# GewelsJI/MVLT

Measured on AMD Instinct MI355X. Metric: image-text pairs/sec/node, PVT-tiny MVLT pre-train step, higher is better.
Workload: dtype bf16

## Files before the change

mvlt_amd/_lib.py:

```python
import ctypes as C
import os

import torch

_HERE = os.path.dirname(os.path.abspath(__file__))
LIB_PATH = os.environ.get("MVLT_HIP_LIB") or os.path.join(_HERE, "libmvlt_hip.so")


class MVLTError(RuntimeError):
    pass


if not os.path.exists(LIB_PATH):
    raise ImportError(f"{LIB_PATH} is missing: build it with `python -m mvlt_amd.build` (hipcc, gfx950). "
                      "mvlt_amd has no CPU or eager fallback.")
lib = C.CDLL(LIB_PATH)

c_int, c_float, c_void_p, c_long = C.c_int, C.c_float, C.c_void_p, C.c_long


class RowMap(C.Structure):
    _fields_ = [(n, c_int) for n in ("mode", "rows_per_batch", "batch_stride", "offset",
                                     "r", "w_in", "tokens_in", "hw_out", "w_out", "c_seg", "h_in")]

# ... 165 lines not shown
        raise ImportError(f"{LIB_PATH} does not export {_name} (include/mvlt_hip_ext.h): stale build? run python -m mvlt_amd.build")
    _fn = getattr(lib, _name)
    _fn.restype, _fn.argtypes = _res, _args

EXT_VERSION = 1
if lib.mvlt_ext_version() != EXT_VERSION:
    raise ImportError(f"extension mismatch: {LIB_PATH} is version {lib.mvlt_ext_version()}, the binding is version {EXT_VERSION} (stale build? run python -m mvlt_amd.build)")

EMA_PROTOTYPES = {
    "mvlt_ema_version": (_i, []),
    "mvlt_ema_update": (_i, [_vp, _vp, _vp, _l, _f, _f, _vp, _vp]),
    "mvlt_ema_update_buffers": (_i, [_vp, _i, _f, _f, _vp]),
}
for _name, (_res, _args) in EMA_PROTOTYPES.items():
    if not hasattr(lib, _name):
        raise ImportError(f"{LIB_PATH} does not export {_name} (include/mvlt_hip_ema.h): stale build? run python -m mvlt_amd.build")
    _fn = getattr(lib, _name)
    _fn.restype, _fn.argtypes = _res, _args

EMA_VERSION = 1
if lib.mvlt_ema_version() != EMA_VERSION:
    raise ImportError(f"EMA entry points mismatch: {LIB_PATH} is version {lib.mvlt_ema_version()}, the binding is version {EMA_VERSION} (stale build? run python -m mvlt_amd.build)")

DT = {torch.bfloat16: 0, torch.float32: 1}


def last_kernel():
    s = lib.mvlt_last_kernel().decode()
    s = s.replace("(anonymous namespace)::", "")
    if s.startswith("void "):
        s = s[5:]
    depth = 0
    for i, ch in enumerate(s):
        depth += ch == "<"
        depth -= ch == ">"
        if ch == "(" and depth == 0:
            return s[:i]
    return s


def check(rc, what):
    if rc != 0:
        raise MVLTError(f"{what} failed ({rc}): {lib.mvlt_last_error().decode()}")


_raw_stream, _cur_device = torch._C._cuda_getCurrentRawStream, torch._C._cuda_getDevice
# ... 25 lines not shown
```

mvlt_amd/build.py:

```python
import concurrent.futures
import os
import subprocess
import sys

HERE = os.path.dirname(os.path.abspath(__file__))
CSRC = os.path.join(HERE, "csrc")
OBJ = os.path.join(HERE, "csrc", "_obj")
LIB = os.path.join(HERE, "libmvlt_hip.so")
ARCH = "gfx950"
FLAGS = ["--offload-arch=" + ARCH, "-O3", "-std=c++17", "-fPIC", "-ffp-contract=fast", "-Wno-unused-result"]
EXTRA = {"mlp.hip": ["-fno-slp-vectorize"]}


def _sources():
    return sorted(f for f in os.listdir(CSRC) if f.endswith(".hip"))


def source_hash():
    import hashlib
    h = hashlib.sha256()
    files = sorted(os.path.join(CSRC, f) for f in os.listdir(CSRC) if f.endswith((".hip", ".h", ".inc")))
    files += [os.path.join(HERE, "..", "include", h) for h in ("mvlt_hip.h", "mvlt_hip_ext.h", "mvlt_hip_ema.h")]
    for f in files:
        h.update(os.path.basename(f).encode())
        h.update(open(f, "rb").read())
    return h.hexdigest()[:16]


def _deps_mtime():
    hdrs = [os.path.join(CSRC, f) for f in os.listdir(CSRC) if f.endswith((".h", ".inc"))]
    hdrs += [os.path.join(HERE, "..", "include", h) for h in ("mvlt_hip.h", "mvlt_hip_ext.h", "mvlt_hip_ema.h")]
    return max(os.path.getmtime(h) for h in hdrs)


def _compile(src, force, verbose):
    s = os.path.join(CSRC, src)
    o = os.path.join(OBJ, src[:-4] + ".o")
    if not force and os.path.exists(o) and os.path.getmtime(o) >= max(os.path.getmtime(s), _deps_mtime()):
        return o
    cmd = ["hipcc", *FLAGS, *EXTRA.get(src, []), "-c", s, "-o", o]
    if verbose:
        print(" ".join(cmd), flush=True)
    r = subprocess.run(cmd, capture_output=True, text=True)
    if r.returncode != 0:
        raise RuntimeError(f"hipcc failed for {src}:\n{r.stdout}\n{r.stderr}")
    return o


def build(force=False, verbose=False):
    os.makedirs(OBJ, exist_ok=True)
    srcs = _sources()
    with concurrent.futures.ThreadPoolExecutor(max_workers=min(6, len(srcs))) as ex:
        objs = list(ex.map(lambda s: _compile(s, force, verbose), srcs))
    if force or not os.path.exists(LIB) or any(os.path.getmtime(o) > os.path.getmtime(LIB) for o in objs):
# ... 12 lines not shown
```

mvlt_amd/csrc/mim.hip:

```cpp
#include "common.h"
#include "../../include/mvlt_hip.h"

namespace {

constexpr int NT = 256;

template <typename TO> __device__ __forceinline__ void store4(TO* p, const f32x4& v);
template <> __device__ __forceinline__ void store4<bf16>(bf16* p, const f32x4& v) {
  st_g<MVLT_NT_MIM>((bf16x4*)p, bf16x4{(bf16)v[0], (bf16)v[1], (bf16)v[2], (bf16)v[3]});
}
template <> __device__ __forceinline__ void store4<float>(float* p, const f32x4& v) { st_g<MVLT_NT_MIM>((f32x4*)p, v); }
template <typename T> __device__ __forceinline__ f32x4 load4(const T* p);
template <> __device__ __forceinline__ f32x4 load4<float>(const float* p) { return *(const f32x4*)p; }
typedef _Float16 f16x4 __attribute__((ext_vector_type(4)));
template <> __device__ __forceinline__ f32x4 load4<_Float16>(const _Float16* p) {
  const f16x4 v = *(const f16x4*)p;
  return f32x4{(float)v[0], (float)v[1], (float)v[2], (float)v[3]};
}
template <> __device__ __forceinline__ f32x4 load4<bf16>(const bf16* p) {
  const bf16x4 v = *(const bf16x4*)p;
  return f32x4{(float)v[0], (float)v[1], (float)v[2], (float)v[3]};
}

typedef _Float16 f16x8 __attribute__((ext_vector_type(8)));
template <typename T> __device__ __forceinline__ void load8(const T* p, float (&v)[8]);
template <> __device__ __forceinline__ void load8<float>(const float* p, float (&v)[8]) {
  const f32x4 a = *(const f32x4*)p, b = *(const f32x4*)(p + 4);
#pragma unroll
  for (int e = 0; e < 4; ++e) { v[e] = a[e]; v[4 + e] = b[e]; }
}
template <> __device__ __forceinline__ void load8<bf16>(const bf16* p, float (&v)[8]) {
  const bf16x8 a = *(const bf16x8*)p;
#pragma unroll
  for (int e = 0; e < 8; ++e) v[e] = (float)a[e];
}
template <> __device__ __forceinline__ void load8<_Float16>(const _Float16* p, float (&v)[8]) {
  const f16x8 a = *(const f16x8*)p;
#pragma unroll
  for (int e = 0; e < 8; ++e) v[e] = (float)a[e];
}
template <typename TO> __device__ __forceinline__ void store8(TO* p, const float (&v)[8]);
template <> __device__ __forceinline__ void store8<float>(float* p, const float (&v)[8]) {
  st_g<MVLT_NT_MIM>((f32x4*)p, f32x4{v[0], v[1], v[2], v[3]});
  st_g<MVLT_NT_MIM>((f32x4*)(p + 4), f32x4{v[4], v[5], v[6], v[7]});
}
template <> __device__ __forceinline__ void store8<_Float16>(_Float16* p, const float (&v)[8]) {
  f16x8 o;
#pragma unroll
  for (int e = 0; e < 8; ++e) o[e] = (_Float16)v[e];
  st_g<MVLT_NT_MIM>((f16x8*)p, o);
}
template <> __device__ __forceinline__ void store8<bf16>(bf16* p, const float (&v)[8]) {
  bf16x8 o;
#pragma unroll
  for (int e = 0; e < 8; ++e) o[e] = (bf16)v[e];
  st_g<MVLT_NT_MIM>((bf16x8*)p, o);
}

template <int MODE>
__global__ __launch_bounds__(NT) void col_reduce_kernel(const float* z, int ldz, const float* dy, int lddy, const float* mean, const float* rstd,
                                                        int M, int C, float* s1, float* s2) {
  extern __shared__ float sm[];
  for (int i = threadIdx.x; i < 2 * C; i += NT) sm[i] = 0.f;
  __syncthreads();
  const int lane = threadIdx.x & 63, wave = threadIdx.x >> 6;
  constexpr int MAXC = 4;
  float a1[MAXC], a2[MAXC], mu[MAXC], rs[MAXC];
#pragma unroll
  for (int k = 0; k < MAXC; ++k) {
    a1[k] = 0.f; a2[k] = 0.f;
    int c = lane + 64 * k;
    mu[k] = (MODE == 1 && c < C) ? mean[c] : 0.f;
    rs[k] = (MODE == 1 && c < C) ? rstd[c] : 0.f;
  }
  for (long row = (long)blockIdx.x * 4 + wave; row < M; row += (long)gridDim.x * 4) {
#pragma unroll
    for (int k = 0; k < MAXC; ++k) {
      int c = lane + 64 * k;
      if (c < C) {
        float zv = z[row * ldz + c];
// ... 954 lines not shown
```

mvlt_amd/mim.py:

```python
import torch

from . import ops
from .params import pool_zeros
from ._lib import conv3map, rowmap

BN_EPS, BN_MOM = 1e-5, 0.1
STAT_COPIES = 16
CONVS = ("reduction1", "reduction2", "reduction3", "conv_upsample1", "conv_upsample2", "conv_upsample3", "conv_upsample4",
         "conv_upsample5", "conv_concat2", "conv_concat3", "conv4")
_NO_BN_FOLD = False


def _z(shape, dev, dtype=torch.float32):
    return pool_zeros(shape, dtype, dev)


def _e(shape, dev, dtype=torch.float32):
    return torch.empty(shape, device=dev, dtype=dtype)


class MimStep:
    def __init__(self, model, x2, x3, x4, sides, training, need_grad):
        self.m, self.S = model, model.store
        self.dt = model.compute_dtype
        self.dev = x2.device
        self.x = (x2, x3, x4)
        self.B = x2.shape[0]
        self.s1, self.s2, self.s3 = sides
        self.M1, self.M2, self.M3 = (self.B * h * w for h, w in sides)
        self.training = training
        self.need_grad = need_grad
        self.rec = {}
        self.nbt = []
# ... 73 lines not shown
        f = self.rec
        f16 = torch.float16 if (self.training and dt == torch.bfloat16) else torch.float32
        r = self.conv_bn("reduction1", x2, C2, x2.shape[1], s1, C2, ch, M1); low = _e((M1, ch), dev, f16); self.norm(r, low, ch)
        r = self.conv_bn("reduction2", x3, C3, x3.shape[1], s2, C3, ch, M2); mid = _e((M2, ch), dev); self.norm(r, mid, ch)
        r = self.conv_bn("reduction3", x4, C4, x4.shape[1], s3, C4, ch, M3); high = _e((M3, ch), dev); self.norm(r, high, ch)
        uph = self.up2(high, ch, s3, ch)
        HW1, HW2 = s1[0] * s1[1], s2[0] * s2[1]
        cat2 = _e((M2, 2 * ch), dev, dt)
        r = self.conv_bn("conv_upsample1", uph, ch, HW2, s2, ch, ch, M2); cu1o = _e((M2, ch), dev); self.norm(r, cu1o, ch)
        a = _e((M2, ch), dev)
        ops.ew_mul(a, ch, cu1o, ch, mid, ch, M=M2, Cdim=ch, out16=cat2, ld16=2 * ch)
        r = self.conv_bn("conv_upsample4", uph, ch, HW2, s2, ch, ch, M2); self.norm(r, y16=cat2[:, ch:], ld16=2 * ch)
        r = self.conv_bn("conv_concat2", cat2, 2 * ch, HW2, s2, 2 * ch, 2 * ch, M2); c = _e((M2, 2 * ch), dev); self.norm(r, c, 2 * ch)
        cat3 = _e((M1, 3 * ch), dev, dt)
        upm = self.up2(mid, ch, s2, ch)
        r = self.conv_bn("conv_upsample2", upm, ch, HW1, s1, ch, ch, M1); cu2o = _e((M1, ch), dev, f16); self.norm(r, cu2o, ch)
        upa = self.up2(a, ch, s2, ch)
        r = self.conv_bn("conv_upsample3", upa, ch, HW1, s1, ch, ch, M1); cu3o = _e((M1, ch), dev, f16); self.norm(r, cu3o, ch)
        ops.ew_mul(None, 0, cu2o, ch, cu3o, ch, low, ch, M=M1, Cdim=ch, out16=cat3, ld16=3 * ch)
        upc = self.up2(c, 2 * ch, s2, 2 * ch)
        r = self.conv_bn("conv_upsample5", upc, 2 * ch, HW1, s1, 2 * ch, 2 * ch, M1); self.norm(r, y16=cat3[:, ch:], ld16=3 * ch)
        d16 = _e((M1, 3 * ch), dev, dt)
        r = self.conv_bn("conv_concat3", cat3, 3 * ch, HW1, s1, 3 * ch, 3 * ch, M1); self.norm(r, y16=d16, ld16=3 * ch)
        e16 = _e((M1, 3 * ch), dev, dt)
        r = self.conv_bn("conv4", d16, 3 * ch, HW1, s1, 3 * ch, 3 * ch, M1); self.norm(r, y16=e16, ld16=3 * ch)
        sc = _e((M1, 3), dev)
        ops.gemm_nt(e16, S.extra["t2i_head.score.0.weight::W"], sc, M1, 3, 3 * ch, 3 * ch, 3 * ch, 3, bias=S.master("t2i_head.score.0.bias"))
        if target is not None:
            acc = pool_zeros((1,), torch.float32, dev)
            ops.upsample_l1_fwd(sc, 3, B, s1[0], s1[1], 3, 8, target, acc)
            out = (acc / target.numel()).reshape(())
            self.sc, self.target = sc, target
        else:
            out = _e((B, 3, 8 * s1[0], 8 * s1[1]), dev)
            ops.upsample_fwd(sc, 3, B, s1[0], s1[1], 3, 8, out, 0, nchw=True)
        if self.nbt:
            torch._foreach_add_(self.nbt, 1)
            self.nbt = []
        if self.need_grad:
            self.keep = dict(low=low, mid=mid, cu1o=cu1o, cu2o=cu2o, cu3o=cu3o, e16=e16)
        else:
            self.rec = {}
        return out

    def bn_conv_bwd(self, name, dy, lddy, dx=None, lddx=0, accumulate=False, dx_map=None, dx_dtype=torch.float32, need_dx=True):
        S, dev, dt = self.S, self.dev, self.dt
        r = self.rec[name]
        p, M, cin, cout = r["p"], r["M"], r["cin"], r["cout"]
        red = _z((2, cout), dev)
        ops.bn_bwd_reduce(dy, lddy, r["z"], cout, r["mean"], r["rstd"], M, cout, red[0], red[1])
        dz = _e((M, cout), dev, dt)
        ops.bn_bwd_apply(dy, lddy, r["z"], cout, r["mean"], r["rstd"], S.master(p + ".1.weight"), red[0], red[1], M, cout, dz, cout,
                         g_beta=S.grad(p + ".1.bias"), g_gamma=S.grad(p + ".1.weight"))
        from .schedule import conv_wgrad
        conv_wgrad(S, p + ".0.weight", dz, r["xin"], M, cout, 9 * cin, cout, r["ld_in"], r["amap"], 9, cin)
        if not need_dx:
            return None
        gmap = conv3map(r["side"][0], r["side"][1], r["side"][0] * r["side"][1], cout)
        if dx is None:
            dx, lddx = _e((M, cin), dev, dx_dtype), cin
        ops.gemm_nt(dz, S.extra[p + ".0.weight::F"], dx, M, cin, 9 * cout, cout, 9 * cout, lddx, a_map=gmap, c_map=dx_map,
                    R=dx if accumulate else None)
        return dx

    def backward(self, dout, sink=None, dgrad=True):
        S, dev, dt, B = self.S, self.dev, self.dt, self.B
        s1, s2, s3, M1, M2, M3 = self.s1, self.s2, self.s3, self.M1, self.M2, self.M3
        ch = 64
        k = self.keep
        dsc_p = _z((M1, 8), dev, dt)
        if getattr(self, "target", None) is not None:
            ops.upsample_l1_bwd(self.sc, 3, B, s1[0], s1[1], 3, 8, self.target, dout.reshape(1).float().contiguous(), dsc_p, 8)
            self.sc = self.target = None
        else:
            dout = dout.contiguous().float()
            ops.upsample_bwd(dout, 0, True, B, s1[0], s1[1], 3, 8, dsc_p, 8)
        ops.gemm_tn(dsc_p, k["e16"], S.grad("t2i_head.score.0.weight").view(3, 3 * ch), M1, 3, 3 * ch, 8, 3 * ch, 3 * ch,
                    colsum=S.grad("t2i_head.score.0.bias"))
        gd = dt if dt == torch.bfloat16 else torch.float32
        de = _e((M1, 3 * ch), dev, gd)
        ops.gemm_nt(dsc_p, S.extra["t2i_head.score.0.weight::T"], de, M1, 3 * ch, 8, 8, 8, 3 * ch)
        dd = self.bn_conv_bwd("conv4", de, 3 * ch, dx_dtype=gd)
        dcat3 = self.bn_conv_bwd("conv_concat3", dd, 3 * ch, dx_dtype=gd)
        dupc = self.bn_conv_bwd("conv_upsample5", dcat3[:, ch:], 3 * ch, dx_dtype=gd)
        dc = _e((M2, 2 * ch), dev)
        ops.upsample_bwd(dupc, 2 * ch, False, B, s2[0], s2[1], 2 * ch, 2, dc, 2 * ch)
        db = dcat3
        dcu2o, dcu3o, dlow = _e((M1, ch), dev, gd), _e((M1, ch), dev, gd), _e((M1, ch), dev, gd)
        ops.ew_mul3_bwd(db, 3 * ch, k["cu2o"], k["cu3o"], k["low"], ch, dcu2o, dcu3o, dlow, M1, ch)
        dcat2 = _z((M2, 2 * ch), dev)
        dupa = self.bn_conv_bwd("conv_upsample3", dcu3o, ch, dx_dtype=gd)
        ops.upsample_bwd(dupa, ch, False, B, s2[0], s2[1], ch, 2, dcat2, 2 * ch, accumulate=True)
        dupm = self.bn_conv_bwd("conv_upsample2", dcu2o, ch, dx_dtype=gd)
        dmid = _e((M2, ch), dev)
        ops.upsample_bwd(dupm, ch, False, B, s2[0], s2[1], ch, 2, dmid, ch)
        self.bn_conv_bwd("conv_concat2", dc, 2 * ch, dx=dcat2, lddx=2 * ch, accumulate=True)
        duph = self.bn_conv_bwd("conv_upsample4", dcat2[:, ch:], 2 * ch)
        dcu1o = _e((M2, ch), dev)
        ops.ew_mul(dcu1o, ch, dcat2, 2 * ch, k["mid"], ch, M=M2, Cdim=ch)
        ops.ew_mul(dmid, ch, dcat2, 2 * ch, k["cu1o"], ch, M=M2, Cdim=ch, accumulate=True)
        self.bn_conv_bwd("conv_upsample1", dcu1o, ch, dx=duph, lddx=ch, accumulate=True)
        dhigh = _e((M3, ch), dev)
        ops.upsample_bwd(duph, ch, False, B, s3[0], s3[1], ch, 2, dhigh, ch)
        grads = []
        for name, dy, x, side in (("reduction1", dlow, self.x[0], s1), ("reduction2", dmid, self.x[1], s2), ("reduction3", dhigh, self.x[2], s3)):
# ... 39 lines not shown
```

mvlt_amd/ops.py:

```python
import ctypes as C

import torch

from . import _lib as L
from ._lib import DT, check, patchmap, ptr, rowmap, stream_ptr

_ID = rowmap()


def gemm_nt(A, B, C_out, M, N, K, lda, ldb, ldc, *, a_map=None, c_map=None, bias=None, act=0, H=None,
            row_scale=None, rows_per_scale=0, R=None, col_sum=None, col_sumsq=None, col_copies=0, split_k=0, post_ln=None):
    assert A.dtype == B.dtype and A.dtype in DT and (C_out.dtype in DT or (C_out.dtype == torch.float16 and col_sum is not None))
    if bias is not None:
        assert bias.dtype == torch.float32
    if row_scale is not None:
        assert row_scale.dtype == torch.float32
    if R is not None:
        assert R.dtype == C_out.dtype or (R.dtype == torch.float32 and C_out.dtype == torch.bfloat16)
    if H is not None:
        assert H.dtype == C_out.dtype
    if col_sum is not None:
        assert col_sum.dtype == torch.float32 and col_sumsq is not None and col_sumsq.dtype == torch.float32
    a = L.GemmNTArgs(A=ptr(A), B=ptr(B), C=ptr(C_out), M=M, N=N, K=K, lda=lda, ldb=ldb, ldc=ldc,
                     dtype=DT[A.dtype], out_dtype=2 if C_out.dtype == torch.float16 else DT[C_out.dtype], a_map=a_map or _ID, c_map=c_map or _ID,
# ... 272 lines not shown

def bn_norm(z, ldz, mean, rstd, gamma, beta, M, Cdim, y32=None, ld32=0, y16=None, ld16=0):
    check(L.lib.mvlt_bn_norm(ptr(z), ldz, ZDT[z.dtype], ptr(mean), ptr(rstd), ptr(gamma), ptr(beta), M, Cdim, ptr(y32), ld32, ZDT[y32.dtype] if y32 is not None else 1, ptr(y16), ld16,
                             DT[y16.dtype] if y16 is not None else 0, stream_ptr()), "mvlt_bn_norm")


def bn_finalize_norm(z, ldz, s, ss, copies, eps, momentum, mean, rstd, running_mean, running_var, gamma, beta, M, Cdim, y32=None, ld32=0, y16=None, ld16=0):
    assert z.dtype == torch.float16 and (y16 is None or y16.dtype == torch.bfloat16)
    check(L.lib.mvlt_bn_finalize_norm(ptr(z), ldz, ptr(s), ptr(ss), copies, eps, momentum, ptr(mean), ptr(rstd), ptr(running_mean), ptr(running_var), ptr(gamma), ptr(beta), M, Cdim,
                                      ptr(y32), ld32, ZDT[y32.dtype] if y32 is not None else 1, ptr(y16), ld16, stream_ptr()), "mvlt_bn_finalize_norm")


def bn_bwd_reduce(dy, lddy, z, ldz, mean, rstd, M, Cdim, s1, s2):
    assert dy.dtype in DT and z.dtype in ZDT
    check(L.lib.mvlt_bn_bwd_reduce(ptr(dy), lddy, ptr(z), ldz, ZDT[z.dtype], ptr(mean), ptr(rstd), M, Cdim, ptr(s1), ptr(s2), DT[dy.dtype], stream_ptr()), "mvlt_bn_bwd_reduce")


def bn_bwd_apply(dy, lddy, z, ldz, mean, rstd, gamma, s1, s2, M, Cdim, dz16, lddz, g_beta=None, g_gamma=None):
    assert dy.dtype in DT and z.dtype in ZDT
    check(L.lib.mvlt_bn_bwd_apply(ptr(dy), lddy, ptr(z), ldz, ZDT[z.dtype], ptr(mean), ptr(rstd), ptr(gamma), ptr(s1), ptr(s2), M, Cdim, ptr(dz16), lddz,
                                  ptr(g_beta), ptr(g_gamma), DT[dz16.dtype], DT[dy.dtype], stream_ptr()), "mvlt_bn_bwd_apply")


def ew_mul3_bwd(dy, lddy, a, b, c, ld, da, db, dc, M, Cdim):
    assert dy.dtype in DT and da.dtype == db.dtype == dc.dtype == dy.dtype and a.dtype == b.dtype == c.dtype and a.dtype in ZDT
    check(L.lib.mvlt_ew_mul3_bwd(ptr(dy), lddy, ptr(a), ptr(b), ptr(c), ld, ZDT[a.dtype], ptr(da), ptr(db), ptr(dc), M, Cdim, DT[dy.dtype], stream_ptr()), "mvlt_ew_mul3_bwd")


def ew_mul(out, ldo, a, lda, b, ldb, c=None, ldc=0, *, M, Cdim, accumulate=False, out16=None, ld16=0):
    assert a.dtype == b.dtype and (c is None or c.dtype == a.dtype) and a.dtype in ZDT
    check(L.lib.mvlt_ew_mul(ptr(out), ldo, ptr(a), lda, ptr(b), ldb, ptr(c), ldc, ZDT[a.dtype], M, Cdim, 1 if accumulate else 0, ptr(out16), ld16,
                            DT[out16.dtype] if out16 is not None else 0, stream_ptr()), "mvlt_ew_mul")


def upsample_fwd(x, ldx, B, H, W, Cdim, scale, out, ldo, nchw=False):
    check(L.lib.mvlt_upsample_fwd(ptr(x), ldx, B, H, W, Cdim, scale, ptr(out), ldo, DT[out.dtype], 1 if nchw else 0, stream_ptr()), "mvlt_upsample_fwd")


def upsample_bwd(dy, lddy, nchw, B, H, W, Cdim, scale, dx, lddx, accumulate=False):
    assert dy.dtype in DT and dx.dtype in DT
    check(L.lib.mvlt_upsample_bwd(ptr(dy), lddy, 1 if nchw else 0, B, H, W, Cdim, scale, ptr(dx), lddx, 1 if accumulate else 0, DT[dx.dtype],
                                  DT[dy.dtype], stream_ptr()), "mvlt_upsample_bwd")


def upsample_l1_ok(W, scale):
    return W <= 64 and (W * scale) % 4 == 0 and W * scale <= 256
# ... 136 lines not shown
```

Before: 13370.

## Fuse conv4 BatchNorm with the 3-channel score projection in forward and backward

Adds kernels that apply the conv4 BatchNorm and project straight to the 3-channel score map, so the bf16 normalized activation (M x 3ch) is never written and no separate GEMM is launched. In backward, the score-weight gradient, the de = dsc*W^T product and the BN reduce/apply are computed together from z and the 3-wide score gradient. This removes materialising and rereading the wide de and e16 tensors. In exchange the normalize and de terms are recomputed inside the reduce and apply kernels, and the path is limited to bf16 training with C <= 256.

```diff
diff --git a/include/mvlt_hip_mim.h b/include/mvlt_hip_mim.h
--- /dev/null
+++ b/include/mvlt_hip_mim.h
@@ -0,0 +1,25 @@
+#ifndef MVLT_HIP_MIM_H
+#define MVLT_HIP_MIM_H
+#include <stdint.h>
+#ifdef __cplusplus
+extern "C" {
+#endif
+
+#define MVLT_MIM_VERSION 1
+int mvlt_mim_version(void);
+
+int mvlt_bn_finalize_norm_score(const void* z, int ldz, const float* sum, const float* sumsq, int copies, float eps, float momentum, float* mean, float* rstd,
+                                float* running_mean, float* running_var, const float* gamma, const float* beta, const void* w, const float* bias,
+                                long M, int C, float* sc, int ldsc, void* stream);
+
+int mvlt_bn_bwd_reduce_score_scratch(long M, int C);
+int mvlt_bn_bwd_reduce_score(const void* z, int ldz, const void* dsc, int lddsc, const void* wt, const float* mean, const float* rstd, const float* gamma,
+                             const float* beta, long M, int C, float* s1, float* s2, float* g_w, float* g_b, float* scratch, long scratch_floats, void* stream);
+
+int mvlt_bn_bwd_apply_score(const void* dsc, int lddsc, const void* wt, const void* z, int ldz, const float* mean, const float* rstd, const float* gamma,
+                            const float* s1, const float* s2, long M, int C, void* dz, int lddz, float* g_beta, float* g_gamma, void* stream);
+
+#ifdef __cplusplus
+}
+#endif
+#endif
diff --git a/mvlt_amd/_lib.py b/mvlt_amd/_lib.py
--- a/mvlt_amd/_lib.py
+++ b/mvlt_amd/_lib.py
@@ -211,6 +211,23 @@
 if lib.mvlt_ema_version() != EMA_VERSION:
     raise ImportError(f"EMA entry points mismatch: {LIB_PATH} is version {lib.mvlt_ema_version()}, the binding is version {EMA_VERSION} (stale build? run python -m mvlt_amd.build)")
 
+MIM_PROTOTYPES = {
+    "mvlt_mim_version": (_i, []),
+    "mvlt_bn_finalize_norm_score": (_i, [_vp, _i, _vp, _vp, _i, _f, _f, _vp, _vp, _vp, _vp, _vp, _vp, _vp, _vp, _l, _i, _vp, _i, _vp]),
+    "mvlt_bn_bwd_reduce_score_scratch": (_i, [_l, _i]),
+    "mvlt_bn_bwd_reduce_score": (_i, [_vp, _i, _vp, _i, _vp, _vp, _vp, _vp, _vp, _l, _i, _vp, _vp, _vp, _vp, _vp, _l, _vp]),
+    "mvlt_bn_bwd_apply_score": (_i, [_vp, _i, _vp, _vp, _i, _vp, _vp, _vp, _vp, _vp, _l, _i, _vp, _i, _vp, _vp, _vp]),
+}
+for _name, (_res, _args) in MIM_PROTOTYPES.items():
+    if not hasattr(lib, _name):
+        raise ImportError(f"{LIB_PATH} does not export {_name} (include/mvlt_hip_mim.h): stale build? run python -m mvlt_amd.build")
+    _fn = getattr(lib, _name)
+    _fn.restype, _fn.argtypes = _res, _args
+
+MIM_VERSION = 1
+if lib.mvlt_mim_version() != MIM_VERSION:
+    raise ImportError(f"MIM score entry points mismatch: {LIB_PATH} is version {lib.mvlt_mim_version()}, the binding is version {MIM_VERSION} (stale build? run python -m mvlt_amd.build)")
+
 DT = {torch.bfloat16: 0, torch.float32: 1}
 
 
diff --git a/mvlt_amd/build.py b/mvlt_amd/build.py
--- a/mvlt_amd/build.py
+++ b/mvlt_amd/build.py
@@ -20,7 +20,7 @@
     import hashlib
     h = hashlib.sha256()
     files = sorted(os.path.join(CSRC, f) for f in os.listdir(CSRC) if f.endswith((".hip", ".h", ".inc")))
-    files += [os.path.join(HERE, "..", "include", h) for h in ("mvlt_hip.h", "mvlt_hip_ext.h", "mvlt_hip_ema.h")]
+    files += [os.path.join(HERE, "..", "include", h) for h in ("mvlt_hip.h", "mvlt_hip_ext.h", "mvlt_hip_ema.h", "mvlt_hip_mim.h")]
     for f in files:
         h.update(os.path.basename(f).encode())
         h.update(open(f, "rb").read())
@@ -29,7 +29,7 @@
 
 def _deps_mtime():
     hdrs = [os.path.join(CSRC, f) for f in os.listdir(CSRC) if f.endswith((".h", ".inc"))]
-    hdrs += [os.path.join(HERE, "..", "include", h) for h in ("mvlt_hip.h", "mvlt_hip_ext.h", "mvlt_hip_ema.h")]
+    hdrs += [os.path.join(HERE, "..", "include", h) for h in ("mvlt_hip.h", "mvlt_hip_ext.h", "mvlt_hip_ema.h", "mvlt_hip_mim.h")]
     return max(os.path.getmtime(h) for h in hdrs)
 
 
diff --git a/mvlt_amd/csrc/mim.hip b/mvlt_amd/csrc/mim.hip
--- a/mvlt_amd/csrc/mim.hip
+++ b/mvlt_amd/csrc/mim.hip
@@ -1,61 +1,10 @@
 #include "common.h"
+#include "mim_vec.h"
 #include "../../include/mvlt_hip.h"
 
 namespace {
 
 constexpr int NT = 256;
-
-template <typename TO> __device__ __forceinline__ void store4(TO* p, const f32x4& v);
-template <> __device__ __forceinline__ void store4<bf16>(bf16* p, const f32x4& v) {
-  st_g<MVLT_NT_MIM>((bf16x4*)p, bf16x4{(bf16)v[0], (bf16)v[1], (bf16)v[2], (bf16)v[3]});
-}
-template <> __device__ __forceinline__ void store4<float>(float* p, const f32x4& v) { st_g<MVLT_NT_MIM>((f32x4*)p, v); }
-template <typename T> __device__ __forceinline__ f32x4 load4(const T* p);
-template <> __device__ __forceinline__ f32x4 load4<float>(const float* p) { return *(const f32x4*)p; }
-typedef _Float16 f16x4 __attribute__((ext_vector_type(4)));
-template <> __device__ __forceinline__ f32x4 load4<_Float16>(const _Float16* p) {
-  const f16x4 v = *(const f16x4*)p;
-  return f32x4{(float)v[0], (float)v[1], (float)v[2], (float)v[3]};
-}
-template <> __device__ __forceinline__ f32x4 load4<bf16>(const bf16* p) {
-  const bf16x4 v = *(const bf16x4*)p;
-  return f32x4{(float)v[0], (float)v[1], (float)v[2], (float)v[3]};
-}
-
-typedef _Float16 f16x8 __attribute__((ext_vector_type(8)));
-template <typename T> __device__ __forceinline__ void load8(const T* p, float (&v)[8]);
-template <> __device__ __forceinline__ void load8<float>(const float* p, float (&v)[8]) {
-  const f32x4 a = *(const f32x4*)p, b = *(const f32x4*)(p + 4);
-#pragma unroll
-  for (int e = 0; e < 4; ++e) { v[e] = a[e]; v[4 + e] = b[e]; }
-}
-template <> __device__ __forceinline__ void load8<bf16>(const bf16* p, float (&v)[8]) {
-  const bf16x8 a = *(const bf16x8*)p;
-#pragma unroll
-  for (int e = 0; e < 8; ++e) v[e] = (float)a[e];
-}
-template <> __device__ __forceinline__ void load8<_Float16>(const _Float16* p, float (&v)[8]) {
-  const f16x8 a = *(const f16x8*)p;
-#pragma unroll
-  for (int e = 0; e < 8; ++e) v[e] = (float)a[e];
-}
-template <typename TO> __device__ __forceinline__ void store8(TO* p, const float (&v)[8]);
-template <> __device__ __forceinline__ void store8<float>(float* p, const float (&v)[8]) {
-  st_g<MVLT_NT_MIM>((f32x4*)p, f32x4{v[0], v[1], v[2], v[3]});
-  st_g<MVLT_NT_MIM>((f32x4*)(p + 4), f32x4{v[4], v[5], v[6], v[7]});
-}
-template <> __device__ __forceinline__ void store8<_Float16>(_Float16* p, const float (&v)[8]) {
-  f16x8 o;
-#pragma unroll
-  for (int e = 0; e < 8; ++e) o[e] = (_Float16)v[e];
-  st_g<MVLT_NT_MIM>((f16x8*)p, o);
-}
-template <> __device__ __forceinline__ void store8<bf16>(bf16* p, const float (&v)[8]) {
-  bf16x8 o;
-#pragma unroll
-  for (int e = 0; e < 8; ++e) o[e] = (bf16)v[e];
-  st_g<MVLT_NT_MIM>((bf16x8*)p, o);
-}
 
 template <int MODE>
 __global__ __launch_bounds__(NT) void col_reduce_kernel(const float* z, int ldz, const float* dy, int lddy, const float* mean, const float* rstd,
diff --git a/mvlt_amd/csrc/mim_score.hip b/mvlt_amd/csrc/mim_score.hip
--- /dev/null
+++ b/mvlt_amd/csrc/mim_score.hip
@@ -0,0 +1,324 @@
+#include "common.h"
+#include "mim_vec.h"
+#include "../../include/mvlt_hip.h"
+#include "../../include/mvlt_hip_mim.h"
+
+namespace {
+
+constexpr int NT = 256;
+constexpr int RWGS = 256;
+
+__device__ __forceinline__ float bf16_round(float x) { return (float)(bf16)x; }
+__device__ __forceinline__ float de_of(float d0, float d1, float d2, float w0, float w1, float w2) { return bf16_round(d0 * w0 + d1 * w1 + d2 * w2); }
+
+template <int KC>
+__global__ __launch_bounds__(NT) void bn_fin_norm_score_kernel(const _Float16* z, int ldz, const float* sum, const float* sumsq, int copies, long Mstat, float eps, float momentum,
+                                                               float* mean, float* rstd, float* running_mean, float* running_var, const float* gamma, const float* beta,
+                                                               const bf16* w, const float* bias, long M, int C, float* sc, int ldsc) {
+  __shared__ __attribute__((aligned(16))) float s_mu[256], s_rs[256];
+  for (int c = threadIdx.x; c < C; c += NT) {
+    float s1 = 0.f, s2 = 0.f;
+    for (int k = 0; k < copies; ++k) { s1 += sum[(long)k * C + c]; s2 += sumsq[(long)k * C + c]; }
+    const float m = s1 / (int)Mstat;
+    const float var = fmaxf(s2 / (int)Mstat - m * m, 0.f);
+    const float r = rsqrtf(var + eps);
+    s_mu[c] = m; s_rs[c] = r;
+    if (blockIdx.x == 0) {
+      mean[c] = m; rstd[c] = r;
+      if (running_mean) {
+        running_mean[c] = (1.f - momentum) * running_mean[c] + momentum * m;
+        const float unb = Mstat > 1 ? var * ((float)(int)Mstat / (float)((int)Mstat - 1)) : var;
+        running_var[c] = (1.f - momentum) * running_var[c] + momentum * unb;
+      }
+    }
+  }
+  __syncthreads();
+  const int lane = threadIdx.x & 63, wave = threadIdx.x >> 6, sub = lane & 7;
+  float mu[KC][8], rs[KC][8], ga[KC][8], be[KC][8], w0[KC][8], w1[KC][8], w2[KC][8];
+  bool on[KC];
+#pragma unroll
+  for (int k = 0; k < KC; ++k) {
+    const int c = (sub + 8 * k) * 8;
+    on[k] = c < C;
+    if (on[k]) {
+      load8<float>(s_mu + c, mu[k]); load8<float>(s_rs + c, rs[k]); load8<float>(gamma + c, ga[k]); load8<float>(beta + c, be[k]);
+      load8<bf16>(w + c, w0[k]); load8<bf16>(w + C + c, w1[k]); load8<bf16>(w + 2 * (long)C + c, w2[k]);
+    } else {
+#pragma unroll
+      for (int e = 0; e < 8; ++e) { mu[k][e] = rs[k][e] = ga[k][e] = be[k][e] = w0[k][e] = w1[k][e] = w2[k][e] = 0.f; }
+    }
+  }
+  const float bj = sub < 3 ? bias[sub] : 0.f;
+  constexpr int RPW = NT / 64 * 8;
+  const long stride = (long)gridDim.x * RPW;
+  for (long rb = (long)blockIdx.x * RPW + wave * 8; rb < M; rb += 2 * stride) {
+    float v[2][KC][8];
+#pragma unroll
+    for (int u = 0; u < 2; ++u) {
+      const long r = rb + u * stride + (lane >> 3);
+#pragma unroll
+      for (int k = 0; k < KC; ++k) {
+        if (on[k] && r < M) load8<_Float16>(z + r * ldz + (sub + 8 * k) * 8, v[u][k]);
+        else {
+#pragma unroll
+          for (int e = 0; e < 8; ++e) v[u][k][e] = 0.f;
+        }
+      }
+    }
+#pragma unroll
+    for (int u = 0; u < 2; ++u) {
+      float a0 = 0.f, a1 = 0.f, a2 = 0.f;
+#pragma unroll
+      for (int k = 0; k < KC; ++k)
+#pragma unroll
+        for (int e = 0; e < 8; ++e) {
+          const float o = bf16_round((v[u][k][e] - mu[k][e]) * rs[k][e] * ga[k][e] + be[k][e]);
+          a0 += o * w0[k][e]; a1 += o * w1[k][e]; a2 += o * w2[k][e];
+        }
+#pragma unroll
+      for (int o = 1; o < 8; o <<= 1) { a0 += __shfl_xor(a0, o); a1 += __shfl_xor(a1, o); a2 += __shfl_xor(a2, o); }
+      const long r = rb + u * stride + (lane >> 3);
+      if (sub < 3 && r < M) sc[r * ldsc + sub] = (sub == 0 ? a0 : sub == 1 ? a1 : a2) + bj;
+    }
+  }
+}
+
+template <int NT>
+__global__ __launch_bounds__(NT) void bn_bwd_reduce_score_kernel(const _Float16* z, int ldz, const bf16* dsc, int lddsc, const bf16* wt, const float* mean, const float* rstd,
+                                                                 long M, int C, float* part, int rows_per_wg) {
+  extern __shared__ float sm[];
+  const int lane = threadIdx.x & 63, wave = threadIdx.x >> 6;
+  const int G = (C + 63) >> 6, g = wave % G, wr = wave / G, R = NT / 64 / G, Cp = G * 64;
+  const int rpp = R * 8;
+  const int tc = g * 64 + (lane & 7) * 8, tr = wr * 8 + (lane >> 3);
+  const bool on = tc < C;
+  float a1[8], a2[8], t0[8], t1[8], t2[8], sd[3] = {0.f, 0.f, 0.f};
+  float mu[8], rs[8], w0[8], w1[8], w2[8];
+#pragma unroll
+  for (int e = 0; e < 8; ++e) { a1[e] = a2[e] = t0[e] = t1[e] = t2[e] = 0.f; mu[e] = rs[e] = w0[e] = w1[e] = w2[e] = 0.f; }
+  if (on) {
+    load8<float>(mean + tc, mu);
+    load8<float>(rstd + tc, rs);
+#pragma unroll
+    for (int e = 0; e < 8; ++e) {
+      const bf16x4 q = *(const bf16x4*)(wt + (long)(tc + e) * 8);
+      w0[e] = (float)q[0]; w1[e] = (float)q[1]; w2[e] = (float)q[2];
+    }
+    const long r0 = (long)blockIdx.x * rows_per_wg;
+    const long r1 = (r0 + rows_per_wg < M) ? r0 + rows_per_wg : M;
+    long r = r0 + tr;
+    constexpr int U = 3;
+    for (; r + (long)(U - 1) * rpp < r1; r += (long)U * rpp) {
+      float zv[U][8];
+      bf16x4 dv[U];
+#pragma unroll
+      for (int u = 0; u < U; ++u) {
+        load8<_Float16>(z + (r + (long)u * rpp) * ldz + tc, zv[u]);
+        dv[u] = *(const bf16x4*)(dsc + (r + (long)u * rpp) * lddsc);
+      }
+#pragma unroll
+      for (int u = 0; u < U; ++u) {
+        const float d0 = (float)dv[u][0], d1 = (float)dv[u][1], d2 = (float)dv[u][2];
+        sd[0] += d0; sd[1] += d1; sd[2] += d2;
+#pragma unroll
+        for (int e = 0; e < 8; ++e) {
+          const float xh = (zv[u][e] - mu[e]) * rs[e], de = de_of(d0, d1, d2, w0[e], w1[e], w2[e]);
+          a1[e] += de; a2[e] += de * xh; t0[e] += d0 * xh; t1[e] += d1 * xh; t2[e] += d2 * xh;
+        }
+      }
+    }
+    for (; r < r1; r += rpp) {
+      float zv[8];
+      load8<_Float16>(z + r * ldz + tc, zv);
+      const bf16x4 dv = *(const bf16x4*)(dsc + r * lddsc);
+      const float d0 = (float)dv[0], d1 = (float)dv[1], d2 = (float)dv[2];
+      sd[0] += d0; sd[1] += d1; sd[2] += d2;
+#pragma unroll
+      for (int e = 0; e < 8; ++e) {
+        const float xh = (zv[e] - mu[e]) * rs[e], de = de_of(d0, d1, d2, w0[e], w1[e], w2[e]);
+        a1[e] += de; a2[e] += de * xh; t0[e] += d0 * xh; t1[e] += d1 * xh; t2[e] += d2 * xh;
+      }
+    }
+  }
+#pragma unroll
+  for (int o = 8; o < 64; o <<= 1) {
+#pragma unroll
+    for (int e = 0; e < 8; ++e) {
+      a1[e] += __shfl_xor(a1[e], o); a2[e] += __shfl_xor(a2[e], o);
+      t0[e] += __shfl_xor(t0[e], o); t1[e] += __shfl_xor(t1[e], o); t2[e] += __shfl_xor(t2[e], o);
+    }
+#pragma unroll
+    for (int j = 0; j < 3; ++j) sd[j] += __shfl_xor(sd[j], o);
+  }
+  float* ss = sm + R * 5 * Cp;
+  if (lane < 8) {
+    float* row = sm + (long)wr * 5 * Cp + tc;
+#pragma unroll
+    for (int e = 0; e < 8; ++e) { row[e] = a1[e]; row[Cp + e] = a2[e]; row[2 * Cp + e] = t0[e]; row[3 * Cp + e] = t1[e]; row[4 * Cp + e] = t2[e]; }
+    if (lane == 0 && g == 0) { ss[wr * 4] = sd[0]; ss[wr * 4 + 1] = sd[1]; ss[wr * 4 + 2] = sd[2]; }
+  }
+  __syncthreads();
+  float* out = part + (long)blockIdx.x * (5 * C + 8);
+  for (int i = threadIdx.x; i < 5 * C; i += NT) {
+    const int q = i / C, c = i - q * C;
+    float t = 0.f;
+    for (int k = 0; k < R; ++k) t += sm[(k * 5 + q) * Cp + c];
+    out[i] = t;
+  }
+  if (threadIdx.x < 3) {
+    float t = 0.f;
+    for (int k = 0; k < R; ++k) t += ss[k * 4 + threadIdx.x];
+    out[5 * C + threadIdx.x] = t;
+  }
+}
+
+__global__ __launch_bounds__(NT) void bn_bwd_reduce_score_finish_kernel(const float* part, int nparts, int C, const float* gamma, const float* beta, float* s1, float* s2,
+                                                                        float* g_w, float* g_b) {
+  __shared__ float f_v[16][16], f_s[16][4];
+  const int k = threadIdx.x & 15, slice = threadIdx.x >> 4;
+  const int v = blockIdx.x * 16 + k, stride = 5 * C + 8;
+  float t = 0.f, ts = 0.f;
+  if (v < 5 * C) {
+#pragma unroll 8
+    for (int p = slice; p < nparts; p += 16) t += part[(long)p * stride + v];
+  }
+  if (k < 3) {
+#pragma unroll 8
+    for (int p = slice; p < nparts; p += 16) ts += part[(long)p * stride + 5 * C + k];
+  }
+  f_v[slice][k] = t;
+  if (k < 4) f_s[slice][k] = ts;
+  __syncthreads();
+  if (threadIdx.x < 16 && v < 5 * C) {
+    float tot = 0.f, s[3] = {0.f, 0.f, 0.f};
+    for (int i = 0; i < 16; ++i) { tot += f_v[i][k]; s[0] += f_s[i][0]; s[1] += f_s[i][1]; s[2] += f_s[i][2]; }
+    const int q = v / C, c = v - q * C;
+    if (q == 0) s1[c] = tot;
+    else if (q == 1) s2[c] = tot;
+    else if (g_w) g_w[(q - 2) * C + c] += gamma[c] * tot + beta[c] * s[q - 2];
+    if (g_b && blockIdx.x == 0 && k < 3) g_b[k] += s[k];
+  }
+}
+
+__global__ __launch_bounds__(NT) void bn_bwd_apply_score_kernel(const bf16* dsc, int lddsc, const bf16* wt, const _Float16* z, int ldz, const float* mean, const float* rstd,
+                                                                const float* gamma, const float* s1, const float* s2, long M, int C, bf16* dz, int lddz,
+                                                                float* g_beta, float* g_gamma) {
+  const int cq = C / 8;
+  const float invM = 1.0f / (float)M;
+  if (g_beta && blockIdx.x == 0)
+    for (int c = threadIdx.x; c < C; c += NT) { g_beta[c] += s1[c]; g_gamma[c] += s2[c]; }
+  const long i0 = (long)blockIdx.x * NT + threadIdx.x;
+  long r = i0 / cq;
+  const int c = (int)(i0 - r * cq) * 8;
+  const long dr = (long)gridDim.x * NT / cq;
+  if (r >= M) return;
+  float mu[8], rs[8], ga[8], t1[8], t2[8], w0[8], w1[8], w2[8];
+  load8<float>(mean + c, mu); load8<float>(rstd + c, rs); load8<float>(gamma + c, ga); load8<float>(s1 + c, t1); load8<float>(s2 + c, t2);
+#pragma unroll
+  for (int e = 0; e < 8; ++e) {
+    const bf16x4 q = *(const bf16x4*)(wt + (long)(c + e) * 8);
+    w0[e] = (float)q[0]; w1[e] = (float)q[1]; w2[e] = (float)q[2];
+  }
+  for (; r < M; r += 2 * dr) {
+    const bool two = r + dr < M;
+    float zv[2][8];
+    bf16x4 dv[2];
+    load8<_Float16>(z + r * ldz + c, zv[0]);
+    dv[0] = *(const bf16x4*)(dsc + r * lddsc);
+    if (two) { load8<_Float16>(z + (r + dr) * ldz + c, zv[1]); dv[1] = *(const bf16x4*)(dsc + (r + dr) * lddsc); }
+#pragma unroll
+    for (int u = 0; u < 2; ++u) {
+      if (u == 1 && !two) break;
+      const float d0 = (float)dv[u][0], d1 = (float)dv[u][1], d2 = (float)dv[u][2];
+      float o[8];
+#pragma unroll
+      for (int e = 0; e < 8; ++e) {
+        const float d = de_of(d0, d1, d2, w0[e], w1[e], w2[e]);
+        const float xh = (zv[u][e] - mu[e]) * rs[e];
+        o[e] = ga[e] * rs[e] * (d - t1[e] * invM - xh * t2[e] * invM);
+      }
+      store8<bf16>(dz + (r + u * dr) * lddz + c, o);
+    }
+  }
+}
+
+inline int grid_for(long work, int cap = 8192) {
+  long g = (work + NT - 1) / NT;
+  if (g > cap) g = cap;
+  if (g < 1) g = 1;
+  return (int)g;
+}
+
+inline bool al16(const void* q) { return ((uintptr_t)q & 15) == 0; }
+inline bool score_shape_ok(const void* z, int ldz, long M, int C) { return z && C > 0 && C % 8 == 0 && C <= 256 && ldz % 8 == 0 && ldz >= C && al16(z) && M > 0 && M < (1L << 31); }
+struct score_red_geo { int nt, rows, grid; };
+inline score_red_geo score_reduce_geo(long M, int C) {
+  const int G = (C + 63) / 64;
+  const int nt = G == 3 ? 768 : 512;
+  const int rpp = (nt / 64 / G) * 8;
+  long rows = (M + RWGS - 1) / RWGS;
+  rows = (rows + 3 * rpp - 1) / (3 * rpp) * (3 * rpp);
+  return {nt, (int)rows, (int)((M + rows - 1) / rows)};
+}
+}
+
+extern "C" int mvlt_mim_version(void) { return MVLT_MIM_VERSION; }
+
+extern "C" int mvlt_bn_finalize_norm_score(const void* z, int ldz, const float* sum, const float* sumsq, int copies, float eps, float momentum, float* mean, float* rstd,
+                                           float* running_mean, float* running_var, const float* gamma, const float* beta, const void* w, const float* bias,
+                                           long M, int C, float* sc, int ldsc, void* stream) {
+  MVLT_REQUIRE(sum && sumsq && mean && rstd && gamma && beta && w && bias && sc && copies >= 1, "mvlt_bn_finalize_norm_score: null pointer, or copies < 1");
+  MVLT_REQUIRE((running_mean == nullptr) == (running_var == nullptr), "mvlt_bn_finalize_norm_score: running_mean and running_var go together");
+  MVLT_REQUIRE(score_shape_ok(z, ldz, M, C) && al16(gamma) && al16(beta) && al16(w) && ldsc >= 3,
+               "mvlt_bn_finalize_norm_score: fp16 z, C a multiple of 8 and <= 256, ldz a multiple of 8, 0 < M < 2^31, z / gamma / beta / w 16-byte aligned, ldsc >= 3");
+  const int KC = (C / 8 + 7) / 8;
+  const int fin_cap = KC == 4 ? 256 : 512;
+  long groups = (M + 63) / 64;
+  const dim3 grid((unsigned)(groups < fin_cap ? groups : fin_cap));
+#define MVLT_FNS(KC_) MVLT_LAUNCH((bn_fin_norm_score_kernel<KC_>), grid, dim3(NT), 0, (hipStream_t)stream, (const _Float16*)z, ldz, sum, sumsq, copies, M, eps, momentum, mean, rstd, \
+                                  running_mean, running_var, gamma, beta, (const bf16*)w, bias, M, C, sc, ldsc)
+  if (KC == 1) MVLT_FNS(1); else if (KC == 2) MVLT_FNS(2); else if (KC == 3) MVLT_FNS(3); else MVLT_FNS(4);
+#undef MVLT_FNS
+  return mvlt_check_launch("mvlt_bn_finalize_norm_score");
+}
+
+extern "C" int mvlt_bn_bwd_reduce_score_scratch(long M, int C) {
+  MVLT_REQUIRE(M > 0 && M < (1L << 31) && C > 0 && C % 8 == 0 && C <= 256, "mvlt_bn_bwd_reduce_score_scratch: 0 < M < 2^31, C a multiple of 8 and <= 256");
+  return score_reduce_geo(M, C).grid * (5 * C + 8);
+}
+
+extern "C" int mvlt_bn_bwd_reduce_score(const void* z, int ldz, const void* dsc, int lddsc, const void* wt, const float* mean, const float* rstd, const float* gamma,
+                                        const float* beta, long M, int C, float* s1, float* s2, float* g_w, float* g_b, float* scratch, long scratch_floats, void* stream) {
+  MVLT_REQUIRE(dsc && wt && mean && rstd && gamma && beta && s1 && s2 && scratch, "mvlt_bn_bwd_reduce_score: null pointer");
+  MVLT_REQUIRE((g_w == nullptr) == (g_b == nullptr), "mvlt_bn_bwd_reduce_score: g_w and g_b go together");
+  MVLT_REQUIRE(score_shape_ok(z, ldz, M, C) && lddsc >= 8 && lddsc % 8 == 0 && al16(dsc) && al16(wt) && al16(mean) && al16(rstd) && al16(scratch),
+               "mvlt_bn_bwd_reduce_score: fp16 z, C a multiple of 8 and <= 256, ldz and lddsc multiples of 8, 0 < M < 2^31, z / dsc / wt / mean / rstd / scratch 16-byte aligned");
+  const score_red_geo geo = score_reduce_geo(M, C);
+  MVLT_REQUIRE(scratch_floats >= (long)geo.grid * (5 * C + 8), "mvlt_bn_bwd_reduce_score: scratch holds %ld floats, %ld needed (mvlt_bn_bwd_reduce_score_scratch)",
+               scratch_floats, (long)geo.grid * (5 * C + 8));
+  const int G = (C + 63) / 64, R = geo.nt / 64 / G;
+  const size_t lds = ((size_t)R * 5 * G * 64 + (size_t)R * 4) * sizeof(float);
+#define MVLT_RS(NT_) MVLT_LAUNCH((bn_bwd_reduce_score_kernel<NT_>), dim3(geo.grid), dim3(NT_), lds, (hipStream_t)stream, (const _Float16*)z, ldz, (const bf16*)dsc, lddsc, \
+                                 (const bf16*)wt, mean, rstd, M, C, scratch, geo.rows)
+  if (geo.nt == 768) MVLT_RS(768); else MVLT_RS(512);
+#undef MVLT_RS
+  int rc = mvlt_check_launch("mvlt_bn_bwd_reduce_score");
+  if (rc != MVLT_OK) return rc;
+  MVLT_LAUNCH(bn_bwd_reduce_score_finish_kernel, dim3((5 * C + 15) / 16), dim3(NT), 0, (hipStream_t)stream, (const float*)scratch, geo.grid, C, gamma, beta, s1, s2, g_w, g_b);
+  return mvlt_check_launch("mvlt_bn_bwd_reduce_score");
+}
+
+extern "C" int mvlt_bn_bwd_apply_score(const void* dsc, int lddsc, const void* wt, const void* z, int ldz, const float* mean, const float* rstd, const float* gamma,
+                                       const float* s1, const float* s2, long M, int C, void* dz, int lddz, float* g_beta, float* g_gamma, void* stream) {
+  MVLT_REQUIRE(dsc && wt && mean && rstd && gamma && s1 && s2 && dz, "mvlt_bn_bwd_apply_score: null pointer");
+  MVLT_REQUIRE((g_beta == nullptr) == (g_gamma == nullptr), "mvlt_bn_bwd_apply_score: g_beta and g_gamma go together");
+  MVLT_REQUIRE(score_shape_ok(z, ldz, M, C) && lddsc >= 8 && lddsc % 8 == 0 && lddz % 8 == 0 && lddz >= C && al16(dsc) && al16(wt) && al16(dz) && al16(mean) && al16(rstd) &&
+               al16(gamma) && al16(s1) && al16(s2),
+               "mvlt_bn_bwd_apply_score: fp16 z, C a multiple of 8 and <= 256, ldz / lddsc / lddz multiples of 8, 0 < M < 2^31, 16-byte aligned tensors");
+  const int cq = C / 8;
+  const int g = grid_for(M * cq);
+  const dim3 grid((unsigned)((g + cq - 1) / cq * cq));
+  MVLT_LAUNCH(bn_bwd_apply_score_kernel, grid, dim3(NT), 0, (hipStream_t)stream, (const bf16*)dsc, lddsc, (const bf16*)wt, (const _Float16*)z, ldz, mean, rstd, gamma, s1, s2, M, C,
+              (bf16*)dz, lddz, g_beta, g_gamma);
+  return mvlt_check_launch("mvlt_bn_bwd_apply_score");
+}
diff --git a/mvlt_amd/csrc/mim_vec.h b/mvlt_amd/csrc/mim_vec.h
--- /dev/null
+++ b/mvlt_amd/csrc/mim_vec.h
@@ -0,0 +1,58 @@
+#pragma once
+#include "common.h"
+
+namespace {
+
+template <typename TO> __device__ __forceinline__ void store4(TO* p, const f32x4& v);
+template <> __device__ __forceinline__ void store4<bf16>(bf16* p, const f32x4& v) {
+  st_g<MVLT_NT_MIM>((bf16x4*)p, bf16x4{(bf16)v[0], (bf16)v[1], (bf16)v[2], (bf16)v[3]});
+}
+template <> __device__ __forceinline__ void store4<float>(float* p, const f32x4& v) { st_g<MVLT_NT_MIM>((f32x4*)p, v); }
+template <typename T> __device__ __forceinline__ f32x4 load4(const T* p);
+template <> __device__ __forceinline__ f32x4 load4<float>(const float* p) { return *(const f32x4*)p; }
+typedef _Float16 f16x4 __attribute__((ext_vector_type(4)));
+template <> __device__ __forceinline__ f32x4 load4<_Float16>(const _Float16* p) {
+  const f16x4 v = *(const f16x4*)p;
+  return f32x4{(float)v[0], (float)v[1], (float)v[2], (float)v[3]};
+}
+template <> __device__ __forceinline__ f32x4 load4<bf16>(const bf16* p) {
+  const bf16x4 v = *(const bf16x4*)p;
+  return f32x4{(float)v[0], (float)v[1], (float)v[2], (float)v[3]};
+}
+
+typedef _Float16 f16x8 __attribute__((ext_vector_type(8)));
+template <typename T> __device__ __forceinline__ void load8(const T* p, float (&v)[8]);
+template <> __device__ __forceinline__ void load8<float>(const float* p, float (&v)[8]) {
+  const f32x4 a = *(const f32x4*)p, b = *(const f32x4*)(p + 4);
+#pragma unroll
+  for (int e = 0; e < 4; ++e) { v[e] = a[e]; v[4 + e] = b[e]; }
+}
+template <> __device__ __forceinline__ void load8<bf16>(const bf16* p, float (&v)[8]) {
+  const bf16x8 a = *(const bf16x8*)p;
+#pragma unroll
+  for (int e = 0; e < 8; ++e) v[e] = (float)a[e];
+}
+template <> __device__ __forceinline__ void load8<_Float16>(const _Float16* p, float (&v)[8]) {
+  const f16x8 a = *(const f16x8*)p;
+#pragma unroll
+  for (int e = 0; e < 8; ++e) v[e] = (float)a[e];
+}
+template <typename TO> __device__ __forceinline__ void store8(TO* p, const float (&v)[8]);
+template <> __device__ __forceinline__ void store8<float>(float* p, const float (&v)[8]) {
+  st_g<MVLT_NT_MIM>((f32x4*)p, f32x4{v[0], v[1], v[2], v[3]});
+  st_g<MVLT_NT_MIM>((f32x4*)(p + 4), f32x4{v[4], v[5], v[6], v[7]});
+}
+template <> __device__ __forceinline__ void store8<_Float16>(_Float16* p, const float (&v)[8]) {
+  f16x8 o;
+#pragma unroll
+  for (int e = 0; e < 8; ++e) o[e] = (_Float16)v[e];
+  st_g<MVLT_NT_MIM>((f16x8*)p, o);
+}
+template <> __device__ __forceinline__ void store8<bf16>(bf16* p, const float (&v)[8]) {
+  bf16x8 o;
+#pragma unroll
+  for (int e = 0; e < 8; ++e) o[e] = (bf16)v[e];
+  st_g<MVLT_NT_MIM>((bf16x8*)p, o);
+}
+
+}
diff --git a/mvlt_amd/mim.py b/mvlt_amd/mim.py
--- a/mvlt_amd/mim.py
+++ b/mvlt_amd/mim.py
@@ -9,6 +9,7 @@
 CONVS = ("reduction1", "reduction2", "reduction3", "conv_upsample1", "conv_upsample2", "conv_upsample3", "conv_upsample4",
          "conv_upsample5", "conv_concat2", "conv_concat3", "conv4")
 _NO_BN_FOLD = False
+_NO_SCORE_FOLD = False
 
 
 def _z(shape, dev, dtype=torch.float32):
@@ -128,10 +129,19 @@
         r = self.conv_bn("conv_upsample5", upc, 2 * ch, HW1, s1, 2 * ch, 2 * ch, M1); self.norm(r, y16=cat3[:, ch:], ld16=3 * ch)
         d16 = _e((M1, 3 * ch), dev, dt)
         r = self.conv_bn("conv_concat3", cat3, 3 * ch, HW1, s1, 3 * ch, 3 * ch, M1); self.norm(r, y16=d16, ld16=3 * ch)
-        e16 = _e((M1, 3 * ch), dev, dt)
-        r = self.conv_bn("conv4", d16, 3 * ch, HW1, s1, 3 * ch, 3 * ch, M1); self.norm(r, y16=e16, ld16=3 * ch)
+        r = self.conv_bn("conv4", d16, 3 * ch, HW1, s1, 3 * ch, 3 * ch, M1)
         sc = _e((M1, 3), dev)
-        ops.gemm_nt(e16, S.extra["t2i_head.score.0.weight::W"], sc, M1, 3, 3 * ch, 3 * ch, 3 * ch, 3, bias=S.master("t2i_head.score.0.bias"))
+        e16 = None
+        if self.training and dt == torch.bfloat16 and r.get("fin") is not None and not _NO_SCORE_FOLD:
+            sm1, sm2, rm, rv = r["fin"]
+            r["fin"] = None
+            ops.bn_finalize_norm_score(r["z"], r["cout"], sm1, sm2, STAT_COPIES, BN_EPS, BN_MOM, r["mean"], r["rstd"], rm, rv, S.master(r["p"] + ".1.weight"),
+                                       S.master(r["p"] + ".1.bias"), S.extra["t2i_head.score.0.weight::W"], S.master("t2i_head.score.0.bias"), M1, r["cout"], sc, 3)
+            r["score"] = True
+        else:
+            e16 = _e((M1, 3 * ch), dev, dt)
+            self.norm(r, y16=e16, ld16=3 * ch)
+            ops.gemm_nt(e16, S.extra["t2i_head.score.0.weight::W"], sc, M1, 3, 3 * ch, 3 * ch, 3 * ch, 3, bias=S.master("t2i_head.score.0.bias"))
         if target is not None:
             acc = pool_zeros((1,), torch.float32, dev)
             ops.upsample_l1_fwd(sc, 3, B, s1[0], s1[1], 3, 8, target, acc)
@@ -149,15 +159,23 @@
             self.rec = {}
         return out
 
-    def bn_conv_bwd(self, name, dy, lddy, dx=None, lddx=0, accumulate=False, dx_map=None, dx_dtype=torch.float32, need_dx=True):
+    def bn_conv_bwd(self, name, dy, lddy, dx=None, lddx=0, accumulate=False, dx_map=None, dx_dtype=torch.float32, need_dx=True, score=None):
         S, dev, dt = self.S, self.dev, self.dt
         r = self.rec[name]
         p, M, cin, cout = r["p"], r["M"], r["cin"], r["cout"]
-        red = _z((2, cout), dev)
-        ops.bn_bwd_reduce(dy, lddy, r["z"], cout, r["mean"], r["rstd"], M, cout, red[0], red[1])
         dz = _e((M, cout), dev, dt)
-        ops.bn_bwd_apply(dy, lddy, r["z"], cout, r["mean"], r["rstd"], S.master(p + ".1.weight"), red[0], red[1], M, cout, dz, cout,
-                         g_beta=S.grad(p + ".1.bias"), g_gamma=S.grad(p + ".1.weight"))
+        if score is not None:
+            wt = S.extra["t2i_head.score.0.weight::T"]
+            red = _e((2, cout), dev)
+            ops.bn_bwd_reduce_score(r["z"], cout, score, 8, wt, r["mean"], r["rstd"], S.master(p + ".1.weight"), S.master(p + ".1.bias"), M, cout, red[0], red[1],
+                                    S.grad("t2i_head.score.0.weight"), S.grad("t2i_head.score.0.bias"), _e((ops.bn_bwd_reduce_score_scratch(M, cout),), dev))
+            ops.bn_bwd_apply_score(score, 8, wt, r["z"], cout, r["mean"], r["rstd"], S.master(p + ".1.weight"), red[0], red[1], M, cout, dz, cout,
+                                   g_beta=S.grad(p + ".1.bias"), g_gamma=S.grad(p + ".1.weight"))
+        else:
+            red = _z((2, cout), dev)
+            ops.bn_bwd_reduce(dy, lddy, r["z"], cout, r["mean"], r["rstd"], M, cout, red[0], red[1])
+            ops.bn_bwd_apply(dy, lddy, r["z"], cout, r["mean"], r["rstd"], S.master(p + ".1.weight"), red[0], red[1], M, cout, dz, cout,
+                             g_beta=S.grad(p + ".1.bias"), g_gamma=S.grad(p + ".1.weight"))
         from .schedule import conv_wgrad
         conv_wgrad(S, p + ".0.weight", dz, r["xin"], M, cout, 9 * cin, cout, r["ld_in"], r["amap"], 9, cin)
         if not need_dx:
@@ -181,12 +199,15 @@
         else:
             dout = dout.contiguous().float()
             ops.upsample_bwd(dout, 0, True, B, s1[0], s1[1], 3, 8, dsc_p, 8)
-        ops.gemm_tn(dsc_p, k["e16"], S.grad("t2i_head.score.0.weight").view(3, 3 * ch), M1, 3, 3 * ch, 8, 3 * ch, 3 * ch,
-                    colsum=S.grad("t2i_head.score.0.bias"))
         gd = dt if dt == torch.bfloat16 else torch.float32
-        de = _e((M1, 3 * ch), dev, gd)
-        ops.gemm_nt(dsc_p, S.extra["t2i_head.score.0.weight::T"], de, M1, 3 * ch, 8, 8, 8, 3 * ch)
-        dd = self.bn_conv_bwd("conv4", de, 3 * ch, dx_dtype=gd)
+        if self.rec["conv4"].get("score"):
+            dd = self.bn_conv_bwd("conv4", None, 0, dx_dtype=gd, score=dsc_p)
+        else:
+            ops.gemm_tn(dsc_p, k["e16"], S.grad("t2i_head.score.0.weight").view(3, 3 * ch), M1, 3, 3 * ch, 8, 3 * ch, 3 * ch,
+                        colsum=S.grad("t2i_head.score.0.bias"))
+            de = _e((M1, 3 * ch), dev, gd)
+            ops.gemm_nt(dsc_p, S.extra["t2i_head.score.0.weight::T"], de, M1, 3 * ch, 8, 8, 8, 3 * ch)
+            dd = self.bn_conv_bwd("conv4", de, 3 * ch, dx_dtype=gd)
         dcat3 = self.bn_conv_bwd("conv_concat3", dd, 3 * ch, dx_dtype=gd)
         dupc = self.bn_conv_bwd("conv_upsample5", dcat3[:, ch:], 3 * ch, dx_dtype=gd)
         dc = _e((M2, 2 * ch), dev)
diff --git a/mvlt_amd/ops.py b/mvlt_amd/ops.py
--- a/mvlt_amd/ops.py
+++ b/mvlt_amd/ops.py
@@ -318,6 +318,54 @@
                                   ptr(g_beta), ptr(g_gamma), DT[dz16.dtype], DT[dy.dtype], stream_ptr()), "mvlt_bn_bwd_apply")
 
 
+def bn_score_ok(Cdim):
+    return Cdim % 8 == 0 and 0 < Cdim <= 256
+
+
+def _score_operands(z, ldz, M, Cdim, dsc=None, lddsc=0, w=None, wt=None):
+    assert z.dtype == torch.float16 and bn_score_ok(Cdim) and ldz >= Cdim and M > 0
+    if dsc is not None:
+        assert dsc.dtype == torch.bfloat16 and lddsc >= 8 and dsc.numel() >= (M - 1) * lddsc + 3
+    if w is not None:
+        assert w.dtype == torch.bfloat16 and w.is_contiguous() and w.numel() >= 3 * Cdim
+    if wt is not None:
+        assert wt.dtype == torch.bfloat16 and wt.is_contiguous() and wt.numel() >= 8 * Cdim
+
+
+def bn_finalize_norm_score(z, ldz, s, ss, copies, eps, momentum, mean, rstd, running_mean, running_var, gamma, beta, w, bias, M, Cdim, sc, ldsc):
+    _score_operands(z, ldz, M, Cdim, w=w)
+    assert s.dtype == ss.dtype == mean.dtype == rstd.dtype == gamma.dtype == beta.dtype == bias.dtype == sc.dtype == torch.float32
+    assert s.numel() >= copies * Cdim and ss.numel() >= copies * Cdim and min(mean.numel(), rstd.numel(), gamma.numel(), beta.numel()) >= Cdim and bias.numel() >= 3
+    assert (running_mean is None) == (running_var is None) and (running_mean is None or running_mean.dtype == running_var.dtype == torch.float32)
+    assert ldsc >= 3 and sc.numel() >= (M - 1) * ldsc + 3
+    check(L.lib.mvlt_bn_finalize_norm_score(ptr(z), ldz, ptr(s), ptr(ss), copies, eps, momentum, ptr(mean), ptr(rstd), ptr(running_mean), ptr(running_var), ptr(gamma), ptr(beta),
+                                            ptr(w), ptr(bias), M, Cdim, ptr(sc), ldsc, stream_ptr()), "mvlt_bn_finalize_norm_score")
+
+
+def bn_bwd_reduce_score_scratch(M, Cdim):
+    n = L.lib.mvlt_bn_bwd_reduce_score_scratch(M, Cdim)
+    check(min(n, 0), "mvlt_bn_bwd_reduce_score_scratch")
+    return n
+
+
+def bn_bwd_reduce_score(z, ldz, dsc, lddsc, wt, mean, rstd, gamma, beta, M, Cdim, s1, s2, g_w, g_b, scratch):
+    _score_operands(z, ldz, M, Cdim, dsc, lddsc, wt=wt)
+    assert mean.dtype == rstd.dtype == gamma.dtype == beta.dtype == s1.dtype == s2.dtype == scratch.dtype == torch.float32
+    assert min(mean.numel(), rstd.numel(), gamma.numel(), beta.numel(), s1.numel(), s2.numel()) >= Cdim and scratch.is_contiguous()
+    assert (g_w is None) == (g_b is None) and (g_w is None or (g_w.dtype == g_b.dtype == torch.float32 and g_w.is_contiguous() and g_w.numel() >= 3 * Cdim and g_b.numel() >= 3))
+    check(L.lib.mvlt_bn_bwd_reduce_score(ptr(z), ldz, ptr(dsc), lddsc, ptr(wt), ptr(mean), ptr(rstd), ptr(gamma), ptr(beta), M, Cdim, ptr(s1), ptr(s2), ptr(g_w), ptr(g_b),
+                                         ptr(scratch), scratch.numel(), stream_ptr()), "mvlt_bn_bwd_reduce_score")
+
+
+def bn_bwd_apply_score(dsc, lddsc, wt, z, ldz, mean, rstd, gamma, s1, s2, M, Cdim, dz16, lddz, g_beta=None, g_gamma=None):
+    _score_operands(z, ldz, M, Cdim, dsc, lddsc, wt=wt)
+    assert mean.dtype == rstd.dtype == gamma.dtype == s1.dtype == s2.dtype == torch.float32 and dz16.dtype == torch.bfloat16
+    assert min(mean.numel(), rstd.numel(), gamma.numel(), s1.numel(), s2.numel()) >= Cdim and lddz >= Cdim and dz16.numel() >= (M - 1) * lddz + Cdim
+    assert (g_beta is None) == (g_gamma is None) and (g_beta is None or (g_beta.dtype == g_gamma.dtype == torch.float32 and min(g_beta.numel(), g_gamma.numel()) >= Cdim))
+    check(L.lib.mvlt_bn_bwd_apply_score(ptr(dsc), lddsc, ptr(wt), ptr(z), ldz, ptr(mean), ptr(rstd), ptr(gamma), ptr(s1), ptr(s2), M, Cdim, ptr(dz16), lddz,
+                                        ptr(g_beta), ptr(g_gamma), stream_ptr()), "mvlt_bn_bwd_apply_score")
+
+
 def ew_mul3_bwd(dy, lddy, a, b, c, ld, da, db, dc, M, Cdim):
     assert dy.dtype in DT and da.dtype == db.dtype == dc.dtype == dy.dtype and a.dtype == b.dtype == c.dtype and a.dtype in ZDT
     check(L.lib.mvlt_ew_mul3_bwd(ptr(dy), lddy, ptr(a), ptr(b), ptr(c), ld, ZDT[a.dtype], ptr(da), ptr(db), ptr(dc), M, Cdim, DT[dy.dtype], stream_ptr()), "mvlt_ew_mul3_bwd")
```

Result: no change. 13440, median of 6 (+0.5%).
